# ATTron/astroz

Measured on AMD Instinct MI355X. Metric: propagations/sec, 13,478 sats x 1,440 times, at 1/2/4/8 MI355X, higher is better.
Workload: dtype f64

## Files before the change

astroz_amd/_native.py:

```python
import ctypes as C
import os

import numpy as np

_HERE = os.path.dirname(os.path.abspath(__file__))
LIB_PATH = os.environ.get("ASTROZ_AMD_LIB") or os.path.join(_HERE, "libastroz_hip.so")

WGS84, WGS72 = 0, 1
OUT_TEME, OUT_ECEF, OUT_GEODETIC, OUT_TOPOCENTRIC = 0, 1, 2, 3
SAT_MAJOR, TIME_MAJOR = 0, 1
OUTPUT_MODES = {"teme": OUT_TEME, "ecef": OUT_ECEF, "geodetic": OUT_GEODETIC, "topocentric": OUT_TOPOCENTRIC}
PASS_DTYPE = np.dtype([("t_rise_min", "<f8"), ("t_culm_min", "<f8"), ("t_set_min", "<f8"), ("max_elevation_rad", "<f8"),
                       ("rise_azimuth_rad", "<f8"), ("set_azimuth_rad", "<f8"), ("flags", "<u4"), ("grid_rise", "<u4"),
                       ("grid_culm", "<u4"), ("grid_set", "<u4")])
PASS_UP_AT_START, PASS_UP_AT_END, PASS_CUT_BY_ERROR = 1, 2, 4
ECLIPSE_DTYPE = np.dtype([("t_entry_min", "<f8"), ("t_exit_min", "<f8"), ("flags", "<u4"), ("grid_entry", "<u4"),
                          ("grid_exit", "<u4"), ("reserved", "<u4")])
ECLIPSE_IN_AT_START, ECLIPSE_IN_AT_END, ECLIPSE_CUT_BY_ERROR = 1, 2, 4
SHADOW_UMBRA, SHADOW_PENUMBRA = 0, 1
SHADOW_KINDS = {"umbra": SHADOW_UMBRA, "penumbra": SHADOW_PENUMBRA}
ACCESS_DTYPE = np.dtype([("t_start_min", "<f8"), ("t_end_min", "<f8"), ("min_range_km", "<f8"), ("flags", "<u4"),
                         ("grid_start", "<u4"), ("grid_end", "<u4"), ("grid_min_range", "<u4")])
ACCESS_OPEN_AT_START, ACCESS_OPEN_AT_END, ACCESS_CUT_BY_ERROR = 1, 2, 4
CONJUNCTION_DTYPE = np.dtype([("t_tca_min", "<f8"), ("miss_km", "<f8"), ("rel_speed_km_s", "<f8"), ("target", "<u4"),
# ... 4 lines not shown
                           ("flags", "<u4"), ("reserved", "<u4")])
COVERAGE_GAP_AT_START, COVERAGE_GAP_AT_END = 1, 2

AZ_ERR_HIP = -200
PATH_ROWS_FAST, PATH_TILES_FAST, PATH_ROWS_GENERIC, PATH_LANE_SAT, PATH_DEEP_ROWS, PATH_QUASI_UNIFORM, PATH_COLS_FAST, PATH_HOST_STEP = 1, 2, 4, 8, 16, 32, 64, 128

EXPORTS = [
    "astroz_version", "astroz_init", "astroz_deinit", "tle_parse", "tle_free",
    "tle_get_satellite_number", "tle_get_epoch", "tle_get_inclination", "tle_get_eccentricity",
    "tle_get_mean_motion", "sgp4_init", "sgp4_free", "sgp4_propagate", "sgp4_propagate_batch",
    "azh_device_count", "azh_last_error", "azh_parse_tle_lines", "azh_constellation_from_tle_text",
    "azh_constellation_from_tle_lines", "azh_constellation_from_elements", "azh_constellation_subset", "azh_constellation_free",
    "azh_num_satellites", "azh_num_sgp4", "azh_num_sdp4", "azh_get_epochs", "azh_get_status",
    "azh_get_field", "azh_propagate_host", "azh_propagate_device", "azh_propagate_device_cached", "azh_propagate_device_window",
    "azh_propagate_jd_host", "azh_synchronize", "azh_propagate_one_host", "azh_set_time_tile", "azh_set_timing", "azh_set_fast_path", "azh_set_tile_kernel", "azh_set_graphs", "azh_set_f32_arithmetic", "azh_set_f32_mode",
    "azh_last_kernel_ms", "azh_last_path", "azh_last_one_stats", "azh_last_window_tiers", "azh_last_window_ecc_tiers", "azh_set_host_copy_threads", "azh_set_host_points", "azh_get_host_points", "azh_selftest_coords", "azh_selftest_host_step", "azh_host_alloc", "azh_host_free", "azh_host_pool_stats", "azh_host_pool_trim", "azh_propagate_device_f32", "azh_propagate_device_cached_f32",
    "azh_screen_target_host", "azh_screen_target_device", "azh_coarse_screen_device", "azh_coarse_screen_host",
    "azh_screen_all_host", "azh_constellation_from_omm_json", "azh_propagate_one_device", "azh_selftest_math",
    "azh_parse_tle_text", "azh_parse_omm_json", "azh_set_parse_threads", "coords_julian_to_gmst",
    "azh_group_create_from_tle_text", "azh_group_create_from_omm_json", "azh_group_free", "azh_group_num_satellites",
    "azh_group_num_devices", "azh_group_padded_rows", "azh_group_get_epochs", "azh_group_propagate_host",
    "azh_group_propagate_allgather", "azh_group_screen_target_host", "azh_group_screen_target_device", "azh_group_shard_size",
    "azh_group_shard_rows", "azh_group_synchronize", "azh_screen_track_device", "coords_eci_to_ecef", "coords_ecef_to_geodetic",
    "orbital_hohmann", "orbital_velocity", "orbital_period", "orbital_escape_velocity",
    "azh_coords_topocentric", "azh_set_observer", "azh_find_passes_host", "azh_find_passes_device",
    "azh_find_passes_stations_host", "azh_find_passes_stations_device",
    "azh_coverage_host", "azh_coverage_device",
    "azh_sun_position_teme", "azh_selftest_sun", "azh_shadow_state", "azh_find_eclipses_host", "azh_find_eclipses_device",
    "azh_line_of_sight", "azh_find_access_host", "azh_find_access_device", "azh_find_access_track_device",
    "azh_closest_approach", "azh_find_conjunctions_host", "azh_find_conjunctions_device",
]
# ... 181 lines not shown
    L.azh_host_alloc.restype = i32
    L.azh_host_free.argtypes = [C.c_void_p]
    L.azh_host_free.restype = None
    L.azh_host_pool_stats.argtypes = [C.POINTER(C.c_size_t), C.POINTER(C.c_size_t)]
    L.azh_host_pool_stats.restype = None
    L.azh_host_pool_trim.argtypes = []
    L.azh_host_pool_trim.restype = None
    L.azh_last_path.argtypes = [vp]
    L.azh_last_path.restype = u32
    L.azh_last_one_stats.argtypes = [vp, vp, vp]
    L.azh_last_one_stats.restype = C.c_int32
    L.azh_last_window_tiers.argtypes = [vp, vp]
    L.azh_last_window_tiers.restype = C.c_int32
    L.azh_last_window_ecc_tiers.argtypes = [vp, vp]
    L.azh_last_window_ecc_tiers.restype = C.c_int32
    L.azh_propagate_device_f32.argtypes = L.azh_propagate_device.argtypes
    L.azh_propagate_device_f32.restype = i32
    L.azh_propagate_device_cached_f32.argtypes = L.azh_propagate_device_cached.argtypes
    L.azh_propagate_device_cached_f32.restype = i32
    L.azh_screen_target_host.argtypes = [vp, vp, sz, vp, sz, dbl, dbl, vp, vp]
    L.azh_screen_target_host.restype = i32
    L.azh_screen_target_device.argtypes = [vp, vp, sz, vp, sz, dbl, dbl, vp, vp, vp]
    L.azh_screen_target_device.restype = i32
    L.azh_screen_track_device.argtypes = [vp, vp, sz, vp, vp, sz, dbl, vp, vp, vp]
    L.azh_screen_track_device.restype = i32
    L.azh_coarse_screen_device.argtypes = [vp, sz, sz, i32, sz, dbl, vp, vp, vp, sz, C.POINTER(sz), vp]
    L.azh_coarse_screen_device.restype = i32
    L.azh_coarse_screen_host.argtypes = [vp, sz, sz, i32, sz, dbl, vp, vp, vp, sz, C.POINTER(sz), i32]
    L.azh_coarse_screen_host.restype = i32
    L.azh_screen_all_host.argtypes = [vp, vp, sz, vp, dbl, vp, vp, sz, C.POINTER(sz)]
# ... 422 lines not shown
        a, b = C.c_uint32(0), C.c_uint32(0)
        check(lib().azh_last_one_stats(self._h, C.byref(a), C.byref(b)), "azh_last_one_stats")
        return int(a.value), int(b.value)


    def last_window_tiers(self):
        cnt = (C.c_uint32 * 4)()
        check(lib().azh_last_window_tiers(self._h, cnt), "azh_last_window_tiers")
        return dict(zip(("general", "eps", "ecc", "rejected"), (int(x) for x in cnt)))

    def last_window_ecc_tiers(self):
        cnt = (C.c_uint32 * 3)()
        check(lib().azh_last_window_ecc_tiers(self._h, cnt), "azh_last_window_ecc_tiers")
        return dict(zip(("e1", "e2", "general"), (int(x) for x in cnt)))


class DeviceGroup:

    def __init__(self, text, devices, grav=WGS72, n_chunks=4):
        b = text.encode() if isinstance(text, str) else bytes(text)
        dv = (C.c_int32 * len(devices))(*devices)
        h = C.c_void_p()
        fn = lib().azh_group_create_from_omm_json if b.lstrip()[:1] in (b"{", b"[") else lib().azh_group_create_from_tle_text
        check(fn(b, len(b), grav, dv, len(devices), n_chunks, C.byref(h)), "azh_group_create")
        self._h = h
        self.n = lib().azh_group_num_satellites(h)
        self.n_devices = lib().azh_group_num_devices(h)
        self.padded_rows = lib().azh_group_padded_rows(h)
        self.epochs = np.empty(self.n)
        check(lib().azh_group_get_epochs(h, self.epochs.ctypes.data), "azh_group_get_epochs")
# ... 289 lines not shown
```

astroz_amd/csrc/astroz_hip.hip:

```cpp
#include "../../include/astroz_hip.h"

#include <hip/hip_runtime.h>
#include <dlfcn.h>
#include <rccl/rccl.h>

#include <algorithm>
#include <atomic>
#include <cmath>
#include <condition_variable>
#include <deque>
#include <map>
#include <cstdio>
#include <cstdlib>
#include <cstring>
#include <mutex>
#include <new>
#include <memory>
#include <string>
#include <thread>
#include <type_traits>
#include <vector>

#include "kernels.h"
#include "passes_kernel.h"
// ... 3077 lines not shown
        f.resize((size_t)pl.n_list * pl.n_seg);
    } catch (const std::bad_alloc &) {
        return AZ_ERR_HIP;
    }
    if (f.empty()) return AZ_OK;
    HIP_TRY(hipMemcpy(f.data(), pl.flag.p, f.size(), hipMemcpyDeviceToHost));
    for (unsigned char v : f) {
        if (!(v & AZ_PLAN_SET)) continue;
        if (!(v & AZ_PLAN_OK)) ++counts[AZH_WINDOW_TIER_REJECTED];
        else if (v & AZ_PLAN_ECC) ++counts[AZH_WINDOW_TIER_ECC];
        else ++counts[((v >> AZ_PLAN_TIER_SHIFT) & AZ_PLAN_TIER_MASK) ? AZH_WINDOW_TIER_EPS : AZH_WINDOW_TIER_GENERAL];
    }
    return AZ_OK;
}

int32_t azh_last_window_ecc_tiers(azh_constellation *c, uint32_t counts[AZH_WINDOW_ECC_COUNTS])
{
    if (!c || !counts) return AZ_ERR_NULL_POINTER;
    for (unsigned k = 0; k < AZH_WINDOW_ECC_COUNTS; ++k) counts[k] = 0;
    if (c->last_plan < 0 || !c->plan[c->last_plan].valid) return AZ_OK;
    const azh_constellation::FastPlan &pl = c->plan[c->last_plan];
    if (set_device(c) != AZ_OK) return AZ_ERR_HIP;
    HIP_TRY(hipDeviceSynchronize());
    std::vector<unsigned char> f;
    try {
        f.resize((size_t)pl.n_list * pl.n_seg);
    } catch (const std::bad_alloc &) {
        return AZ_ERR_HIP;
    }
    if (f.empty()) return AZ_OK;
// ... 712 lines not shown
```

astroz_amd/csrc/fast_step.h:

```cpp
#pragma once
#include <type_traits>

#include "propagate_device.h"

#define AZ_FASTK_COLD(X)                                                                                     \
    X(cc1) X(d2) X(d3) X(d4) X(nl2) X(nl3) X(nl4) X(nl5) X(eta) X(omgcof) X(xmcof) X(xd) X(bc4) X(bc5) X(ecb) X(sab)
#define AZ_FASTK_HOT(X)                                                                                      \
    X(aycof) X(xlcof) X(xnodcf) X(sinio) X(cosio) X(k_mrt) X(k_c2u) X(k_su) X(k_node) X(k_inc) X(x1mth2) X(k_rv) \
    X(sdA) X(cdA) X(sdW) X(cdW) X(tc) X(sdU) X(cdU) X(tmid) X(nodedot) X(sOc) X(cOc)
enum FastCold {
#define X(n) FC_##n,
    AZ_FASTK_COLD(X)
#undef X
    FC_NUM
};
#define AZ_FASTK_DELTA(X) X(mdot) X(argpdot) X(udot)
enum FastColdX {
    FCX_first_ = FC_NUM - 1,
#define X(n) FCX_##n,
    AZ_FASTK_DELTA(X)
#undef X
    FCX_NUM
};
#define AZ_DELTA_MAX 4.0e-6
// ... 330 lines not shown
    const double inv_pl = inv_am / (1.0 - el2);
    const double temp2 = g.half_j2 * inv_pl * inv_pl;
    ok &= temp2 <= AZ_FAST_TEMP2;
    const double a_nd = fma(fabs(k.k_node_), temp2, fma(fabs(k.nodedot_), 0.5 * fabs(t_b - t_a) + dmax, fabs(k.xnodcf_) * T * T));
    ok &= a_nd <= AZ_ROT_MED;
    if (!ok) return -1;
    if (ECC) return el <= AZ_ETIER_E1_MAX ? (int)AZ_ETIER_E1 : (el <= AZ_ETIER_E2_MAX ? (int)AZ_ETIER_E2 : (int)AZ_TIER_GENERAL);
    return eps <= AZ_TIER_EPS_MAX ? AZ_TIER_EPS : AZ_TIER_GENERAL;
}
template <bool ECC>
AZ_DEVICE bool az_fast_window_ok(const FastK &k, const AzGrav &g, double t_a, double t_b, double dmax = 0.0)
{
    return az_fast_window_tier<ECC>(k, g, t_a, t_b, dmax) >= 0;
}

#ifndef AZ_FAST_PROBE
#define AZ_FAST_PROBE(name, value)
#endif
#ifndef AZ_FAST_PROBE_KEPLER
#define AZ_FAST_PROBE_KEPLER(name, value)
#endif

template <bool VEL, bool ECC = false, int DELTA = 0, int TIER = AZ_TIER_GENERAL, class K = FastK, class RC = RotCoefLit>
AZ_DEVICE bool az_sgp4_fast_step(const K &k, const AzGrav &g, const RC &rk, double t, FastCarry &st, double r[3],
                                  double v[3], double dl = 0.0)
{
    az_pair_advance<K::SCALAR>(st.sA, st.cA, k.sdA(), k.cdA());
    az_pair_advance<K::SCALAR>(st.sW, st.cW, k.sdW(), k.cdW());
    az_pair_advance<K::SCALAR>(st.sU, st.cU, k.sdU(), k.cdU());
    double sA = st.sA, cA = st.cA, sW = st.sW, cW = st.cW;
    if constexpr ((DELTA == 1 && ECC) || DELTA == 2) {
        const double a = k.mdot() * dl, b = k.argpdot() * dl;
        if constexpr (DELTA == 2 && ECC) {
            double pa, qa;
            az_pq_16th(a, rk, pa, qa);
            az_rot_apply2(sA, cA, pa, qa);
        } else if constexpr (DELTA == 2) {
            az_rotate_tiny2(sA, cA, a, rk);
        } else {
            sA = fma(st.cA, a, st.sA); cA = fma(-st.sA, a, st.cA);
        }
        if constexpr (DELTA == 2 && ECC) az_rotate_tiny2(sW, cW, b, rk);
        else { sW = fma(st.cW, b, st.sW); cW = fma(-st.sW, b, st.cW); }
    }
    const double t2 = t * t;
    constexpr bool E1 = ECC && TIER == AZ_ETIER_E1, E2 = ECC && TIER == AZ_ETIER_E2;

    const double dm = fma(k.eta(), cA, 1.0);
    const double th = fma(k.xmcof(), dm * dm * dm, fma(k.omgcof(), t, -k.xd()));
    const double tempa = fma(-t, fma(t, fma(t, fma(t, k.d4(), k.d3()), k.d2()), k.cc1()), 1.0);
    const double dtc = t - k.tc();
    double nl = fma(k.nl2() * dtc, dtc, t2 * (t * fma(t, fma(t, k.nl5(), k.nl4()), k.nl3())));
    if constexpr (DELTA != 0) nl = fma(k.udot(), dl, nl);
    bool bad = false;
    double p, q;
    if (E1) az_fpq_small(th, rk, p, q);
    else if (ECC) az_pq_16th(th, rk, p, q);
    else az_pq_ecc_scaled(th, rk, p, q);
    const double smm = fma(cA, p, fma(sA, q, sA));
    const double sw = fma(-cW, p, fma(sW, q, sW));
    const double cw = fma(sW, p, fma(cW, q, cW));
    const double em = fma(-k.bc5(), smm, fma(-k.bc4(), t, k.ecb()));
    AZ_FAST_PROBE(th, th)
    AZ_FAST_PROBE(em, em)

    const double sqrt_am = k.sab() * fabs(tempa);
    const double am = sqrt_am * sqrt_am;
    const double omem2 = fma(-em, em, 1.0);
    const double R = az_rcp(sqrt_am * omem2);
    const double ra = R * omem2;
    const double temp = ra * R;

    const double axnl = em * cw;
    const double aynl = fma(em, sw, temp * k.aycof());
    double s = st.sU, c = st.cU;
    {
        const double eps = fma(temp * k.xlcof(), axnl, nl);
        AZ_FAST_PROBE(eps, eps)
        if constexpr (!ECC && TIER >= AZ_TIER_EPS) az_rotate_tiny2(s, c, eps, rk);
        else {
            az_pq_16th(eps, rk, p, q);
            az_rot_apply2(s, c, p, q);
        }
    }

    const double el2 = fma(axnl, axnl, aynl * aynl);
// ... 93 lines not shown

    const double est = esine * inv_1pb;
    const double sinu = inv_ome * (s - fma(axnl, est, aynl));
    const double cosu = inv_ome * (c + fma(aynl, est, -axnl));
    const double sin2u = (sinu + sinu) * cosu;
    const double cos2u = fma(-2.0 * sinu, sinu, 1.0);

    const double inv_am = ra * ra;
    const double rl = am * ome;
    const double inv_pl = inv_am * inv_omel2;
    const double temp1 = g.half_j2 * inv_pl;
    const double temp2 = temp1 * inv_pl;

    const double mrt = fma(rl, fma(k.k_mrt() * temp2, betal, 1.0), k.k_c2u() * temp1 * cos2u);
    const double t2s = temp2 * sin2u;
    const double a_nd = fma(k.k_node(), t2s, fma(k.nodedot(), t - k.tmid(), k.xnodcf() * t2));
    AZ_FAST_PROBE(a_nd, a_nd)
    double ssu = sinu, csu = cosu, sn = k.sOc(), cn = k.cOc(), si = k.sinio(), ci = k.cosio();
    az_rotate_tiny2(ssu, csu, k.k_su() * t2s, rk);
    az_pq_16th(a_nd, rk, p, q);
    az_rot_apply2(sn, cn, p, q);
    az_rotate_tiny2(si, ci, k.k_inc() * temp2 * cos2u, rk);

    const double xmx = -sn * ci, xmy = cn * ci;
    const double rs = mrt * g.radius_km;
    const double ra_s = rs * ssu, ra_c = rs * csu;
    r[0] = fma(xmx, ra_s, cn * ra_c);
    r[1] = fma(xmy, ra_s, sn * ra_c);
    r[2] = si * ra_s;
    if (VEL) {
        const double rv = ra * g.vkmpersec;
// ... 12 lines not shown
```

astroz_amd/csrc/kernels.h:

```cpp
#pragma once
#include <hip/hip_runtime.h>

#include <type_traits>

#include "init_device.h"
#include "propagate_device.h"
#include "fast_step.h"
#include "fast_step_f32.h"

#ifndef AZ_BLOCK
#define AZ_BLOCK 256
#endif
#ifndef AZ_PROP_FAST
#define AZ_PROP_FAST 1
#endif
#ifndef AZ_MIN_WAVES
#define AZ_MIN_WAVES 1
#endif
#ifndef AZ_ROWS_WAVES
#define AZ_ROWS_WAVES 3
#endif
#ifndef AZ_DEEP_WAVES
#define AZ_DEEP_WAVES 2
#endif
// ... 58 lines not shown
    const unsigned *redo_static;
    AzGrav g;
};
enum { AZ_ROW_NEAR = 0, AZ_ROW_COPY = 1, AZ_ROW_ZERO = 2 };
enum { AZ_PLAN_sOc, AZ_PLAN_cOc, AZ_PLAN_sdU, AZ_PLAN_cdU, AZ_PLAN_s1U, AZ_PLAN_c1U, AZ_PLAN_NUM };
#define AZ_PLAN_OK 1u
#define AZ_PLAN_TC 2u
#define AZ_PLAN_TIER_SHIFT 2
#define AZ_PLAN_TIER_MASK 1u
#define AZ_PLAN_ETIER_MASK 3u
#ifndef AZ_ROWS_ETIERS
#define AZ_ROWS_ETIERS 1
#endif
#define AZ_PLAN_ECC 16u
#define AZ_PLAN_SET 32u

template <class T>
__device__ __forceinline__ void az_put3(T *o, const double r[3])
{
    o[0] = (T)r[0];
    o[1] = (T)r[1];
    o[2] = (T)r[2];
}
typedef double az_d2s __attribute__((ext_vector_type(2), aligned(8)));
typedef float az_f3s __attribute__((ext_vector_type(3), aligned(4)));
#ifndef AZ_ROWS_NT
#define AZ_ROWS_NT 1
#endif
__device__ __forceinline__ void az_put3_stream(double *o, const double r[3])
{
// ... 464 lines not shown
    az_load_fast(a.el, a.n_pad, s, fl, a.inc, 0, k0);
    const double dt_mult = ecc ? 64.0 : a.dt_mult;
    if (dt_mult == 128.0) az_double_increments(k0);
    az_fast_window(a.el, a.n_pad, s, w_a, w_b, dt_mult * a.step, k0);
    az_load_fast(a.el, a.n_pad, s, fl, a.inc, 1, k1);
    az_fast_window(a.el, a.n_pad, s, w_a, w_b, a.step, k1);
    int tier = ecc ? az_fast_window_tier<true>(k0, a.g, w_a, w_b, a.delta_max) : az_fast_window_tier<false>(k0, a.g, w_a, w_b, a.delta_max);
    if (ecc && (AZ_ROWS_ETIERS == 0 || (AZ_ROWS_ETIERS == 2 && tier == AZ_ETIER_E2))) tier = min(tier, (int)AZ_TIER_GENERAL);
    bool ok = tier >= 0;
    if (!ecc && AZ_FLAG_ECLASS(fl) != 0) ok = false;
    if (!ecc && a.f32_mixed && !az_fast32p_window_ok(k0, w_a, w_b)) ok = false;
    const size_t at = (size_t)seg * a.n_list + slot;
    double *w = a.win + at * AZ_PLAN_NUM;
    w[AZ_PLAN_sOc] = k0.sOc_; w[AZ_PLAN_cOc] = k0.cOc_; w[AZ_PLAN_sdU] = k0.sdU_; w[AZ_PLAN_cdU] = k0.cdU_;
    w[AZ_PLAN_s1U] = k1.sdU_; w[AZ_PLAN_c1U] = k1.cdU_;
    a.flag[at] = (unsigned char)((ok ? AZ_PLAN_OK | ((unsigned)tier << AZ_PLAN_TIER_SHIFT) : 0u) | (k0.tc_ != 0.0 ? AZ_PLAN_TC : 0u) |
                                 (ecc ? AZ_PLAN_ECC : 0u) | AZ_PLAN_SET);
    if (!ok) {
        const unsigned k = atomicAdd(a.redo_static, 1u);
        a.redo_items[3 * (size_t)k + 0] = slot;
        a.redo_items[3 * (size_t)k + 1] = t_lo;
        a.redo_items[3 * (size_t)k + 2] = t_hi;
    }
}
__global__ void k_plan_arm(unsigned *redo_static, unsigned *c0, unsigned *c1)
{
    if (threadIdx.x == 0 && blockIdx.x == 0) *c0 = *c1 = *redo_static;
}
template <class K>
__device__ __forceinline__ bool az_plan_window(const PropArgs &p, unsigned seg, unsigned slot, double w_a, double w_b, K &k0, unsigned *tier = nullptr)
{
    const size_t at = (size_t)seg * p.plan_stride + slot;
    const double *w = p.plan_win + at * AZ_PLAN_NUM;
    const unsigned f = p.plan_flag[at];
    k0.tmid_ = 0.5 * (w_a + w_b);
    k0.tc_ = (f & AZ_PLAN_TC) ? k0.tmid_ : 0.0;
    k0.sOc_ = w[AZ_PLAN_sOc]; k0.cOc_ = w[AZ_PLAN_cOc]; k0.sdU_ = w[AZ_PLAN_sdU]; k0.cdU_ = w[AZ_PLAN_cdU];
    if (tier) *tier = (f >> AZ_PLAN_TIER_SHIFT) & ((f & AZ_PLAN_ECC) ? AZ_PLAN_ETIER_MASK : AZ_PLAN_TIER_MASK);
    return (f & AZ_PLAN_OK) != 0;
}

AZ_DEVICE double az_uniform(double x)
{
#ifdef AZ_HOST_EMUL
    return x;
#else
    return __hiloint2double(__builtin_amdgcn_readfirstlane(__double2hiint(x)),
                            __builtin_amdgcn_readfirstlane(__double2loint(x)));
#endif
}
AZ_DEVICE float az_uniform32(float x)
{
#ifdef AZ_HOST_EMUL
// ... 230 lines not shown
__global__ void __launch_bounds__(64, FRAME >= 2 ? 4 : (ECC ? AZ_ROWSF_ECC_WAVES : (FRAME == 1 || DELTA == 2 ? 5 : AZ_ROWSF_WAVES))) k_rows_fast(PropArgs p)
{
    typedef typename std::conditional<SINK == AZ_SINK_F32, float, double>::type out_t;
    const unsigned lane = threadIdx.x;
    const unsigned row = az_list_slot(p);
    [[maybe_unused]] const AzObserver obs = FRAME == 3 ? *p.obs : AzObserver{};
    if (row >= az_list_end(p)) return;
    const unsigned s = p.list[row];
    if (SINK != AZ_SINK_SCREEN && ((p.mask != nullptr && p.mask[s] == 0) || s < p.row_lo || s >= p.row_hi)) return;
    const unsigned t_lo = blockIdx.y * p.tile;
    if (t_lo >= p.n_times) return;
    const unsigned t_hi = min(t_lo + p.tile, p.n_times);
    unsigned base = t_lo;
    bool window_ok;
    unsigned tier = AZ_TIER_GENERAL;
    double best_d2 = __builtin_inf();
    unsigned best_t = 0xffffffffu;
    {
        __shared__ __attribute__((aligned(16))) double cold_lds[AZ_FAST_TABLE];
        __shared__ __attribute__((aligned(16))) out_t rows_stage[AZ_ROWS_LDS_STORE ? 2 * 64 * 3 : 4];
        const double off = az_uniform(p.offsets ? p.offsets[s] : 0.0);
        const double *__restrict__ rec = p.fast_rec + (size_t)s * FR_NUM;
        az_fill_fast_table(cold_lds, rec, lane);
        const size_t out_row = p.rows_compact ? (size_t)p.ecc_row0 + row : (size_t)s;
        out_t *prow = SINK == AZ_SINK_SCREEN ? nullptr : reinterpret_cast<out_t *>(p.pos) + out_row * p.n_times * 3;
        out_t *vrow = VEL ? reinterpret_cast<out_t *>(p.vel) + out_row * p.n_times * 3 : nullptr;
        const bool staged = AZ_ROWS_LDS_STORE && SINK != AZ_SINK_SCREEN &&
                            (((reinterpret_cast<size_t>(prow) | (VEL ? reinterpret_cast<size_t>(vrow) : 0)) & 15u) == 0);
        FastKBcast k;
        {
            const double w_a = fma((double)t_lo, p.uniform_step, p.grid_t0 + off), w_b = fma((double)(t_hi - 1), p.uniform_step, p.grid_t0 + off);
            window_ok = az_plan_window(p, blockIdx.y, row + p.redo_slot0, w_a, w_b, k, &tier);
            if (!window_ok) return;
            az_fast_rec_hot(rec, k);
            az_wave_lds_fence();
            if (DELTA && k.tc_ != 0.0 && lane == 0) cold_lds[FCX_udot] = fma(2.0 * rec[FC_nl2], k.tc_, rec[FCX_udot]);
        }
        typedef typename std::conditional<DELTA == 2, double, float>::type dl_t;
        __shared__ dl_t dl_lds[DELTA ? AZ_DELTA_SEG : 1];
        if (DELTA) {
            const dl_t *src = DELTA == 2 ? reinterpret_cast<const dl_t *>(p.delta64) : reinterpret_cast<const dl_t *>(p.delta);
#pragma unroll
            for (unsigned j = lane; j < AZ_DELTA_SEG; j += 64) dl_lds[j] = src[t_lo + j];
        }
        az_wave_lds_fence();
        const double step = p.uniform_step;
        const double t_first = p.grid_t0 + off;
        FastCarry fc;
        az_seed_fast_rec(rec, rec[FC_nl2], fma((double)(t_lo + lane) - 64.0, step, t_first), k.tc_, fc,
                         McLds{cold_lds + FCX_NUM + RC_NUM});
        __shared__ double gst_lds[FRAME ? 2 * AZ_FRAME_SEG : 2];
        if (FRAME) {
#pragma unroll
            for (unsigned j = lane; j < AZ_FRAME_SEG; j += 64) {
                const unsigned jj = min(t_lo + j, p.n_times - 1);
                gst_lds[2 * j] = p.sin_g[jj];
                gst_lds[2 * j + 1] = p.cos_g[jj];
            }
            az_wave_lds_fence();
        }
        AzRowSink sink{};
        if constexpr (SINK != AZ_SINK_SCREEN) sink = az_row_sink(prow, vrow, p.n_times);
        auto run = [&](auto tier_c, const unsigned t_end) __attribute__((always_inline)) {
        constexpr int TIER = decltype(tier_c)::value;
#pragma unroll 1
        for (; window_ok && base < t_end; base += 64) {
            const unsigned i = base + lane;
            const bool live = i < t_hi;
            double t = fma((double)i, step, t_first), dl = 0.0;
            if (DELTA) {
                dl = (double)dl_lds[i - t_lo];
                t += dl;
            }
            const double *cold_now = az_opaque_lds(cold_lds);
            k.cold = cold_now;
            const RotCoefLds rk{cold_now + FCX_NUM};
            double r[3], v[3];
#if defined(AZ_ABLATE) && AZ_ABLATE == 2
            r[0] = t; r[1] = t + 1.0; r[2] = t + 2.0; v[0] = t + 3.0; v[1] = t + 4.0; v[2] = t + 5.0;
#else
            const bool bad = az_sgp4_fast_step<VEL, ECC, DELTA, TIER>(k, p.g, rk, t, fc, r, v, dl);
            if (az_any(bad && live)) break;
#endif
            if (SINK == AZ_SINK_SCREEN) {
                const double *q = p.screen_target + (size_t)(live ? i : t_hi - 1) * 3;
                const double dx = q[0] - r[0], dy = q[1] - r[1], dz = q[2] - r[2];
                const double d2 = fma(dx, dx, fma(dy, dy, dz * dz));
                if (live && d2 < best_d2) {
                    best_d2 = d2;
                    best_t = i;
                }
                continue;
            }
            if (FRAME) {
                if (((base - t_lo) & (AZ_FRAME_SEG - 1u)) == 0u && base != t_lo) {
                    az_wave_lds_fence();
// ... 6 lines not shown
                    az_wave_lds_fence();
                }
                const unsigned jj = (i - t_lo) & (AZ_FRAME_SEG - 1u);
                const double sg = gst_lds[2 * jj], cg = gst_lds[2 * jj + 1];
                az_to_ecef(r, sg, cg);
                if (VEL) az_to_ecef(v, sg, cg);
                if (FRAME == 2) az_ecef_to_geodetic(r);
                if (FRAME == 3) az_topocentric<VEL>(r, v, obs);
            }
#if defined(AZ_ABLATE) && AZ_ABLATE == 1
            if (!(live && (r[0] + r[1] + r[2] + (VEL ? v[0] + v[1] + v[2] : 0.0)) == 1.2345e300)) continue;
#endif
            az_rows_store<VEL>(staged, base + 64 <= t_hi, live, lane, rows_stage, prow, vrow, base, r, v, sink);
        }
        };
        if constexpr (AZ_ROWS_TIERS && !ECC && FRAME == 0) run(std::integral_constant<int, AZ_TIER_EPS>(), tier == AZ_TIER_EPS ? t_hi : t_lo);
        if constexpr (AZ_ROWS_ETIERS && ECC && FRAME == 0 && DELTA != 2) {
            run(std::integral_constant<int, AZ_ETIER_E1>(), tier == AZ_ETIER_E1 ? t_hi : t_lo);
            if constexpr (AZ_ROWS_ETIERS == 1) run(std::integral_constant<int, AZ_ETIER_E2>(), tier == AZ_ETIER_E2 ? t_hi : t_lo);
        }
        run(std::integral_constant<int, AZ_TIER_GENERAL>(), t_hi);
    }
    if (SINK == AZ_SINK_SCREEN) {
        az_wave_argmin(best_d2, best_t);
        if (lane == 0) {
            p.part_d2[(size_t)blockIdx.y * p.plan_stride + row + p.redo_slot0] = best_d2;
            p.part_t[(size_t)blockIdx.y * p.plan_stride + row + p.redo_slot0] = best_t;
        }
    }
    if (ECC && base < t_hi && lane == 0) {
        const unsigned k = atomicAdd(p.redo_count, 1u);
        p.redo_items[3 * (size_t)k + 0] = row + p.redo_slot0;
        p.redo_items[3 * (size_t)k + 1] = base;
        p.redo_items[3 * (size_t)k + 2] = t_hi;
    }
}
// ... 910 lines not shown
```

bindings/zig/astroz_hip.zig:

```

pub const HipError = error{
    BadTleLength,
    BadChecksum,
    DeepSpaceNotSupported,
    InvalidEccentricity,
    SatelliteDecayed,
    ValueError,
    OutOfMemory,
    NullPointer,
    NotInitialized,
    DeviceFailure,
    Unknown,
};

pub fn check(rc: i32) HipError!void {
    return switch (rc) {
        0 => {},
        -1 => HipError.BadTleLength,
        -2 => HipError.BadChecksum,
        -10 => HipError.DeepSpaceNotSupported,
        -11 => HipError.InvalidEccentricity,
        -12 => HipError.SatelliteDecayed,
        -20 => HipError.ValueError,
        -100 => HipError.OutOfMemory,
// ... 77 lines not shown
pub extern "c" fn azh_set_f32_arithmetic(h: ?*Handle, enabled: i32) i32;
pub extern "c" fn azh_set_fast_path(h: ?*Handle, enabled: i32) i32;
pub extern "c" fn azh_set_tile_kernel(h: ?*Handle, enabled: i32) i32;
pub extern "c" fn azh_set_graphs(h: ?*Handle, enabled: i32) i32;
pub extern "c" fn azh_set_host_points(n: usize) void;
pub extern "c" fn azh_get_host_points() usize;
pub extern "c" fn azh_set_host_copy_threads(n: i32) void;
pub extern "c" fn azh_host_alloc(bytes: usize, out: *?*anyopaque) i32;
pub extern "c" fn azh_host_free(p: ?*anyopaque) void;
pub extern "c" fn azh_host_pool_stats(live_bytes: ?*usize, free_bytes: ?*usize) void;
pub extern "c" fn azh_host_pool_trim() void;
pub extern "c" fn azh_last_path(h: ?*const Handle) u32;
pub extern "c" fn azh_last_one_stats(h: ?*Handle, n_segments: ?*u32, n_handed_over: ?*u32) i32;
pub extern "c" fn azh_last_window_tiers(h: ?*Handle, counts: *[4]u32) i32;
pub extern "c" fn azh_last_window_ecc_tiers(h: ?*Handle, counts: *[3]u32) i32;
pub extern "c" fn azh_propagate_one_device(h: ?*Handle, sat_index: usize, d_tsince_min: [*]const f64, n: usize, d_pos: [*]f64,
    d_vel: ?[*]f64, d_err: ?[*]u8, stream: ?*anyopaque) i32;
pub extern "c" fn azh_selftest_math(x: [*]const f64, n: usize, out6n: [*]f64, device: i32) i32;
pub extern "c" fn azh_selftest_host_step(el: [*]const f64, n_pad: usize, sat: usize, flags: u32, grav: i32, tsince_min: [*]const f64, n: usize,
    out6n: [*]f64, err: ?[*]u8) i32;
pub extern "c" fn azh_selftest_coords(op: i32, in: *const [4]f64, out: *[5]f64) i32;

pub extern "c" fn coords_julian_to_gmst(jd: f64) f64;
pub extern "c" fn coords_eci_to_ecef(eci: *const [3]f64, gmst: f64, ecef: *[3]f64) void;
pub extern "c" fn coords_ecef_to_geodetic(ecef: *const [3]f64, lla: *[3]f64) void;
pub extern "c" fn azh_coords_topocentric(r_teme: *const [3]f64, v_teme: ?*const [3]f64, gmst: f64, observer_lla: *const [3]f64,
    aer: *[3]f64, aer_rate: ?*[3]f64) void;

pub const OUT_TOPOCENTRIC: i32 = 3;
pub const Pass = extern struct {
// ... 132 lines not shown
```

include/astroz_hip.h:

```cpp
#ifndef ASTROZ_HIP_H
#define ASTROZ_HIP_H

#include <stddef.h>
#include <stdint.h>

#ifdef __cplusplus
extern "C" {
#endif

enum {
    AZ_OK = 0,
    AZ_ERR_BAD_TLE_LENGTH = -1,
    AZ_ERR_BAD_CHECKSUM = -2,
    AZ_ERR_DEEP_SPACE_NOT_SUPPORTED = -10,
    AZ_ERR_INVALID_ECCENTRICITY = -11,
    AZ_ERR_SATELLITE_DECAYED = -12,
    AZ_ERR_VALUE = -20,
    AZ_ERR_ALLOC_FAILED = -100,
    AZ_ERR_NULL_POINTER = -101,
    AZ_ERR_NOT_INITIALIZED = -102,
    AZ_ERR_HIP = -200,
    AZ_ERR_UNKNOWN = -999
};

// ... 282 lines not shown
#define AZH_PATH_QUASI_UNIFORM 32u
#define AZH_PATH_HOST_STEP 128u
uint32_t azh_last_path(const azh_constellation *c);
int32_t azh_last_one_stats(azh_constellation *c, uint32_t *n_segments, uint32_t *n_handed_over);
#define AZH_WINDOW_TIER_GENERAL 0
#define AZH_WINDOW_TIER_EPS 1
#define AZH_WINDOW_TIER_ECC 2
#define AZH_WINDOW_TIER_REJECTED 3
#define AZH_WINDOW_TIER_COUNTS 4
int32_t azh_last_window_tiers(azh_constellation *c, uint32_t counts[AZH_WINDOW_TIER_COUNTS]);
#define AZH_WINDOW_ECC_E1 0
#define AZH_WINDOW_ECC_E2 1
#define AZH_WINDOW_ECC_GENERAL 2
#define AZH_WINDOW_ECC_COUNTS 3
int32_t azh_last_window_ecc_tiers(azh_constellation *c, uint32_t counts[AZH_WINDOW_ECC_COUNTS]);

#ifdef __cplusplus
}
#endif
#endif
```

Baseline: 97.61 billion.

## Replace per-step secular polynomials with per-64-step quadratic block expansions in LDS

For near-circular windows that pass an analytic error-bound check, the planner sets a new block flag. The rows kernel then precomputes Taylor coefficients for each 64-step block around its midpoint (am, ra, temp, nl, node, theta and eccentricity terms) and stores them in LDS. Each lane evaluates low-degree polynomials in its offset instead of the full per-time polynomials, reciprocals and divisions. This cuts per-step arithmetic, but adds an LDS table, extra template instantiations and a tolerance-bounded approximation error. A query API counts how many windows took the block path.

```diff
diff --git a/astroz_amd/_native.py b/astroz_amd/_native.py
--- a/astroz_amd/_native.py
+++ b/astroz_amd/_native.py
@@ -42,7 +42,7 @@
     "azh_num_satellites", "azh_num_sgp4", "azh_num_sdp4", "azh_get_epochs", "azh_get_status",
     "azh_get_field", "azh_propagate_host", "azh_propagate_device", "azh_propagate_device_cached", "azh_propagate_device_window",
     "azh_propagate_jd_host", "azh_synchronize", "azh_propagate_one_host", "azh_set_time_tile", "azh_set_timing", "azh_set_fast_path", "azh_set_tile_kernel", "azh_set_graphs", "azh_set_f32_arithmetic", "azh_set_f32_mode",
-    "azh_last_kernel_ms", "azh_last_path", "azh_last_one_stats", "azh_last_window_tiers", "azh_last_window_ecc_tiers", "azh_set_host_copy_threads", "azh_set_host_points", "azh_get_host_points", "azh_selftest_coords", "azh_selftest_host_step", "azh_host_alloc", "azh_host_free", "azh_host_pool_stats", "azh_host_pool_trim", "azh_propagate_device_f32", "azh_propagate_device_cached_f32",
+    "azh_last_kernel_ms", "azh_last_path", "azh_last_one_stats", "azh_last_window_tiers", "azh_last_window_ecc_tiers", "azh_last_window_blocks", "azh_set_host_copy_threads", "azh_set_host_points", "azh_get_host_points", "azh_selftest_coords", "azh_selftest_host_step", "azh_host_alloc", "azh_host_free", "azh_host_pool_stats", "azh_host_pool_trim", "azh_propagate_device_f32", "azh_propagate_device_cached_f32",
     "azh_screen_target_host", "azh_screen_target_device", "azh_coarse_screen_device", "azh_coarse_screen_host",
     "azh_screen_all_host", "azh_constellation_from_omm_json", "azh_propagate_one_device", "azh_selftest_math",
     "azh_parse_tle_text", "azh_parse_omm_json", "azh_set_parse_threads", "coords_julian_to_gmst",
@@ -254,6 +254,8 @@
     L.azh_last_window_tiers.restype = C.c_int32
     L.azh_last_window_ecc_tiers.argtypes = [vp, vp]
     L.azh_last_window_ecc_tiers.restype = C.c_int32
+    L.azh_last_window_blocks.argtypes = [vp, vp]
+    L.azh_last_window_blocks.restype = C.c_int32
     L.azh_propagate_device_f32.argtypes = L.azh_propagate_device.argtypes
     L.azh_propagate_device_f32.restype = i32
     L.azh_propagate_device_cached_f32.argtypes = L.azh_propagate_device_cached.argtypes
@@ -706,6 +708,11 @@
         check(lib().azh_last_window_ecc_tiers(self._h, cnt), "azh_last_window_ecc_tiers")
         return dict(zip(("e1", "e2", "general"), (int(x) for x in cnt)))
 
+    def last_window_blocks(self):
+        n = C.c_uint32(0)
+        check(lib().azh_last_window_blocks(self._h, C.byref(n)), "azh_last_window_blocks")
+        return int(n.value)
+
 
 class DeviceGroup:
 
diff --git a/astroz_amd/csrc/astroz_hip.hip b/astroz_amd/csrc/astroz_hip.hip
--- a/astroz_amd/csrc/astroz_hip.hip
+++ b/astroz_amd/csrc/astroz_hip.hip
@@ -3115,6 +3115,27 @@
     return AZ_OK;
 }
 
+int32_t azh_last_window_blocks(azh_constellation *c, uint32_t *n_block_windows)
+{
+    if (!c || !n_block_windows) return AZ_ERR_NULL_POINTER;
+    *n_block_windows = 0;
+    if (c->last_plan < 0 || !c->plan[c->last_plan].valid) return AZ_OK;
+    const azh_constellation::FastPlan &pl = c->plan[c->last_plan];
+    if (set_device(c) != AZ_OK) return AZ_ERR_HIP;
+    HIP_TRY(hipDeviceSynchronize());
+    std::vector<unsigned char> f;
+    try {
+        f.resize((size_t)pl.n_list * pl.n_seg);
+    } catch (const std::bad_alloc &) {
+        return AZ_ERR_HIP;
+    }
+    if (f.empty()) return AZ_OK;
+    HIP_TRY(hipMemcpy(f.data(), pl.flag.p, f.size(), hipMemcpyDeviceToHost));
+    for (unsigned char v : f)
+        if ((v & (AZ_PLAN_SET | AZ_PLAN_OK | AZ_PLAN_ECC | AZ_PLAN_BLK)) == (AZ_PLAN_SET | AZ_PLAN_OK | AZ_PLAN_BLK)) ++*n_block_windows;
+    return AZ_OK;
+}
+
 int32_t azh_last_window_ecc_tiers(azh_constellation *c, uint32_t counts[AZH_WINDOW_ECC_COUNTS])
 {
     if (!c || !counts) return AZ_ERR_NULL_POINTER;
diff --git a/astroz_amd/csrc/fast_step.h b/astroz_amd/csrc/fast_step.h
--- a/astroz_amd/csrc/fast_step.h
+++ b/astroz_amd/csrc/fast_step.h
@@ -368,17 +368,123 @@
     return az_fast_window_tier<ECC>(k, g, t_a, t_b, dmax) >= 0;
 }
 
+enum FastBlk { FB_am0, FB_am1, FB_am2, FB_ra0, FB_ra1, FB_ra2, FB_T0, FB_T1, FB_T2, FB_Tw, FB_nl0, FB_nl1, FB_nl2, FB_nl3,
+               FB_n0, FB_n1, FB_n2, FB_th0, FB_em0, FB_NUM };
+#define AZ_BLK_MAX 12
+#define AZ_BLK_TOL 2.0e-14
+struct NoBlock {
+    static constexpr bool ON = false;
+    AZ_MEMBER double x() const { return 0.0; }
+    AZ_MEMBER double operator()(int) const { return 0.0; }
+    AZ_MEMBER NoBlock after(double) const { return *this; }
+};
+struct FastBlock {
+    static constexpr bool ON = true;
+    const double *c;
+    double x_;
+    AZ_MEMBER double x() const { return x_; }
+    AZ_MEMBER double operator()(int j) const { return c[j]; }
+    AZ_MEMBER FastBlock after(double dep) const
+    {
+#ifndef AZ_HOST_EMUL
+        typedef __attribute__((address_space(3))) const double lds_cdouble;
+        lds_cdouble *q = (lds_cdouble *)c;
+        asm volatile("" : "+v"(q) : "v"(dep));
+        return FastBlock{(const double *)q, x_};
+#else
+        (void)dep;
+        return *this;
+#endif
+    }
+};
+template <class K, class W>
+AZ_DEVICE void az_fast_block_coefs(const K &k, double tb, W write)
+{
+    const double d2 = k.d2(), d3 = k.d3(), d4 = k.d4(), cc1 = k.cc1();
+    const double P = fma(-tb, fma(tb, fma(tb, fma(tb, d4, d3), d2), cc1), 1.0);
+    const double P1 = -fma(tb, fma(tb, fma(tb, 4.0 * d4, 3.0 * d3), 2.0 * d2), cc1);
+    const double P2 = -fma(tb, fma(tb, 12.0 * d4, 6.0 * d3), 2.0 * d2);
+    const double sab = k.sab(), S = sab * sab;
+    const double sq = sab * fabs(P);
+    write(FB_am0, sq * sq);
+    write(FB_am1, 2.0 * S * P * P1);
+    write(FB_am2, S * fma(P, P2, P1 * P1));
+    const double ra0 = az_rcp(sq);
+    const double iP = ra0 * sab, u = P1 * iP;
+    write(FB_ra0, ra0);
+    write(FB_ra1, -ra0 * u);
+    write(FB_ra2, ra0 * fma(u, u, -0.5 * P2 * iP));
+    const double bc4 = k.bc4();
+    const double e0 = fma(-bc4, tb, k.ecb());
+    const double gm = az_rcp(fma(-e0, e0, 1.0));
+    const double T0 = ra0 * ra0 * gm;
+    write(FB_T0, T0);
+    const double sg = bc4 * gm, es = e0 * sg;
+    write(FB_T1, -2.0 * T0 * (u + es));
+    write(FB_T2, T0 * fma(fma(3.0 * e0, e0, 1.0) * sg, sg, fma(4.0 * u, es, fma(3.0 * u, u, -P2 * iP))));
+    write(FB_Tw, -2.0 * k.bc5() * e0 * T0 * gm);
+    const double n2 = k.nl2(), n3 = k.nl3(), n4 = k.nl4(), n5 = k.nl5(), dc = tb - k.tc(), tb2 = tb * tb;
+    write(FB_nl0, fma(n2 * dc, dc, tb2 * (tb * fma(tb, fma(tb, n5, n4), n3))));
+    write(FB_nl1, fma(2.0 * n2, dc, tb2 * fma(tb, fma(tb, 5.0 * n5, 4.0 * n4), 3.0 * n3)));
+    write(FB_nl2, fma(tb, fma(tb, fma(tb, 10.0 * n5, 6.0 * n4), 3.0 * n3), n2));
+    write(FB_nl3, fma(tb, fma(tb, 10.0 * n5, 4.0 * n4), n3));
+    const double nd = k.nodedot(), xn = k.xnodcf();
+    write(FB_n0, fma(nd, tb - k.tmid(), xn * tb2));
+    write(FB_n1, fma(2.0 * xn, tb, nd));
+    write(FB_n2, xn);
+    write(FB_th0, fma(k.omgcof(), tb, -k.xd()));
+    write(FB_em0, e0);
+}
+
+enum { BQ_am, BQ_ra, BQ_T, BQ_nl, BQ_nd, BQ_NUM };
+AZ_DEVICE bool az_fast_window_blocks(const FastK &k, double t_a, double t_b, double h0, double dmax, double bnd[BQ_NUM])
+{
+    const double h = h0 + dmax;
+    const double Tb = fmax(fabs(t_a), fabs(t_b)) + h;
+    const double c1 = fabs(k.cc1_), a2 = fabs(k.d2_), a3 = fabs(k.d3_), a4 = fabs(k.d4_);
+    const double da = Tb * fma(Tb, fma(Tb, fma(Tb, a4, a3), a2), c1);
+    const double D1 = fma(Tb, fma(Tb, fma(Tb, 4.0 * a4, 3.0 * a3), 2.0 * a2), c1);
+    const double D2 = fma(Tb, fma(Tb, 12.0 * a4, 6.0 * a3), 2.0 * a2);
+    const double D3 = fma(Tb, 24.0 * a4, 6.0 * a3);
+    const double Pmax = 1.0 + da, iP = 1.0 / (1.0 - da), iP2 = iP * iP, iP3 = iP2 * iP;
+    const double b4 = fabs(k.bc4_), b5 = fabs(k.bc5_);
+    const double emx = fabs(k.ecb_) + fma(b4, Tb, b5);
+    bool ok = (da <= 0.5) & (emx <= 0.9);
+    const double h3 = h * h * h * (1.0 / 6.0);
+    bnd[BQ_am] = fma(fma(6.0 * D1, D2, 2.0 * Pmax * D3) * iP2, h3, 2.0e-15);
+    bnd[BQ_ra] = fma(fma(6.0 * D1 * D1 * D1, iP2 * iP2, fma(6.0 * D1 * D2, iP3, D3 * iP2)) * Pmax, h3, 2.0e-15);
+    const double iS = 1.0 / (k.sab_ * k.sab_);
+    const double A0 = iP2 * iS, A1 = 2.0 * D1 * iP3 * iS, A2 = fma(6.0 * D1 * D1, iP2 * iP2, 2.0 * D2 * iP3) * iS;
+    const double F0 = 1.0 / fma(-emx, emx, 1.0), F1 = 2.0 * emx * F0 * F0, F2 = fma(6.0 * emx, emx, 2.0) * F0 * F0 * F0;
+    const double A3 = fma(24.0 * D1 * D1 * D1, iP2 * iP3, fma(18.0 * D1 * D2, iP2 * iP2, 2.0 * D3 * iP3)) * iS;
+    const double F3 = 24.0 * emx * fma(emx, emx, 1.0) * F0 * F0 * F0 * F0;
+    const double T3 = fma(A3, F0, b4 * fma(3.0 * A2, F1, b4 * fma(3.0 * A1, F2, A0 * F3 * b4)));
+    const double dTw = b5 * fma(A1, F1, A0 * F2 * b4);
+    const double errT = fma(T3, h3, fma(dTw, h, 0.5 * A0 * F2 * b5 * b5)) + 3.0e-15 * A0 * F0;
+    bnd[BQ_T] = errT * fmax(fabs(k.aycof_), fabs(k.xlcof_) * emx);
+    const double n4 = fabs(k.nl4_), n5 = fabs(k.nl5_), h2 = h * h;
+    bnd[BQ_nl] = fma(h2 * h2, fma(5.0 * n5, Tb, n4) + n5 * h, 2.0e-16);
+    bnd[BQ_nd] = 2.0e-16;
+#pragma unroll
+    for (int q = 0; q < BQ_NUM; ++q) ok &= bnd[q] <= AZ_BLK_TOL;
+    return ok;
+}
+
 #ifndef AZ_FAST_PROBE
 #define AZ_FAST_PROBE(name, value)
 #endif
 #ifndef AZ_FAST_PROBE_KEPLER
 #define AZ_FAST_PROBE_KEPLER(name, value)
 #endif
-
-template <bool VEL, bool ECC = false, int DELTA = 0, int TIER = AZ_TIER_GENERAL, class K = FastK, class RC = RotCoefLit>
+#ifndef AZ_FAST_PROBE_BLOCK
+#define AZ_FAST_PROBE_BLOCK(name, value)
+#endif
+
+template <bool VEL, bool ECC = false, int DELTA = 0, int TIER = AZ_TIER_GENERAL, class K = FastK, class RC = RotCoefLit, class B = NoBlock>
 AZ_DEVICE bool az_sgp4_fast_step(const K &k, const AzGrav &g, const RC &rk, double t, FastCarry &st, double r[3],
-                                  double v[3], double dl = 0.0)
-{
+                                  double v[3], double dl = 0.0, const B &b = B())
+{
+    static_assert(!B::ON || (!ECC && DELTA <= 1), "the block form: near-circular bodies, exact and tight grids");
     az_pair_advance<K::SCALAR>(st.sA, st.cA, k.sdA(), k.cdA());
     az_pair_advance<K::SCALAR>(st.sW, st.cW, k.sdW(), k.cdW());
     az_pair_advance<K::SCALAR>(st.sU, st.cU, k.sdU(), k.cdU());
@@ -401,11 +507,16 @@
     constexpr bool E1 = ECC && TIER == AZ_ETIER_E1, E2 = ECC && TIER == AZ_ETIER_E2;
 
     const double dm = fma(k.eta(), cA, 1.0);
-    const double th = fma(k.xmcof(), dm * dm * dm, fma(k.omgcof(), t, -k.xd()));
-    const double tempa = fma(-t, fma(t, fma(t, fma(t, k.d4(), k.d3()), k.d2()), k.cc1()), 1.0);
+    double th, tempa = 1.0, nl = 0.0;
+    if constexpr (B::ON) {
+        th = fma(k.xmcof(), dm * dm * dm, fma(k.omgcof(), b.x(), b(FB_th0)));
+    } else {
+    th = fma(k.xmcof(), dm * dm * dm, fma(k.omgcof(), t, -k.xd()));
+    tempa = fma(-t, fma(t, fma(t, fma(t, k.d4(), k.d3()), k.d2()), k.cc1()), 1.0);
     const double dtc = t - k.tc();
-    double nl = fma(k.nl2() * dtc, dtc, t2 * (t * fma(t, fma(t, k.nl5(), k.nl4()), k.nl3())));
-    if constexpr (DELTA != 0) nl = fma(k.udot(), dl, nl);
+    nl = fma(k.nl2() * dtc, dtc, t2 * (t * fma(t, fma(t, k.nl5(), k.nl4()), k.nl3())));
+    }
+    if constexpr (DELTA != 0 && !B::ON) nl = fma(k.udot(), dl, nl);
     bool bad = false;
     double p, q;
     if (E1) az_fpq_small(th, rk, p, q);
@@ -414,16 +525,29 @@
     const double smm = fma(cA, p, fma(sA, q, sA));
     const double sw = fma(-cW, p, fma(sW, q, sW));
     const double cw = fma(sW, p, fma(cW, q, cW));
-    const double em = fma(-k.bc5(), smm, fma(-k.bc4(), t, k.ecb()));
+    const double em = fma(-k.bc5(), smm, B::ON ? fma(-k.bc4(), b.x(), b(FB_em0)) : fma(-k.bc4(), t, k.ecb()));
     AZ_FAST_PROBE(th, th)
     AZ_FAST_PROBE(em, em)
 
+    double am = 0.0, ra = 0.0, temp;
+    if constexpr (B::ON) {
+        temp = fma(b(FB_Tw), smm, fma(b.x(), fma(b.x(), b(FB_T2), b(FB_T1)), b(FB_T0)));
+        nl = fma(b.x(), fma(b.x(), fma(b.x(), b(FB_nl3), b(FB_nl2)), b(FB_nl1)), b(FB_nl0));
+        if constexpr (DELTA != 0) nl = fma(k.udot(), dl, nl);
+        am = fma(b.x(), fma(b.x(), b(FB_am2), b(FB_am1)), b(FB_am0));
+        ra = fma(b.x(), fma(b.x(), b(FB_ra2), b(FB_ra1)), b(FB_ra0));
+    } else {
     const double sqrt_am = k.sab() * fabs(tempa);
-    const double am = sqrt_am * sqrt_am;
+    am = sqrt_am * sqrt_am;
     const double omem2 = fma(-em, em, 1.0);
     const double R = az_rcp(sqrt_am * omem2);
-    const double ra = R * omem2;
-    const double temp = ra * R;
+    ra = R * omem2;
+    temp = ra * R;
+    }
+    AZ_FAST_PROBE_BLOCK(temp, temp)
+    AZ_FAST_PROBE_BLOCK(nl, nl)
+    AZ_FAST_PROBE_BLOCK(am, am)
+    AZ_FAST_PROBE_BLOCK(ra, ra)
 
     const double axnl = em * cw;
     const double aynl = fma(em, sw, temp * k.aycof());
@@ -547,7 +671,15 @@
 
     const double mrt = fma(rl, fma(k.k_mrt() * temp2, betal, 1.0), k.k_c2u() * temp1 * cos2u);
     const double t2s = temp2 * sin2u;
-    const double a_nd = fma(k.k_node(), t2s, fma(k.nodedot(), t - k.tmid(), k.xnodcf() * t2));
+    double nd;
+    if constexpr (B::ON) {
+        const B b3 = b.after(ome);
+        nd = fma(b.x(), fma(b3(FB_n2), b.x(), b3(FB_n1)), b3(FB_n0));
+    } else {
+        nd = fma(k.nodedot(), t - k.tmid(), k.xnodcf() * t2);
+    }
+    AZ_FAST_PROBE_BLOCK(nd, nd)
+    const double a_nd = fma(k.k_node(), t2s, nd);
     AZ_FAST_PROBE(a_nd, a_nd)
     double ssu = sinu, csu = cosu, sn = k.sOc(), cn = k.cOc(), si = k.sinio(), ci = k.cosio();
     az_rotate_tiny2(ssu, csu, k.k_su() * t2s, rk);
diff --git a/astroz_amd/csrc/kernels.h b/astroz_amd/csrc/kernels.h
--- a/astroz_amd/csrc/kernels.h
+++ b/astroz_amd/csrc/kernels.h
@@ -96,6 +96,10 @@
 #endif
 #define AZ_PLAN_ECC 16u
 #define AZ_PLAN_SET 32u
+#define AZ_PLAN_BLK 64u
+#ifndef AZ_ROWS_BLOCKS
+#define AZ_ROWS_BLOCKS 1
+#endif
 
 template <class T>
 __device__ __forceinline__ void az_put3(T *o, const double r[3])
@@ -590,8 +594,13 @@
     double *w = a.win + at * AZ_PLAN_NUM;
     w[AZ_PLAN_sOc] = k0.sOc_; w[AZ_PLAN_cOc] = k0.cOc_; w[AZ_PLAN_sdU] = k0.sdU_; w[AZ_PLAN_cdU] = k0.cdU_;
     w[AZ_PLAN_s1U] = k1.sdU_; w[AZ_PLAN_c1U] = k1.cdU_;
+    bool blk = false;
+    if (AZ_ROWS_BLOCKS && ok && !ecc && tile <= 64u * AZ_BLK_MAX && a.delta_max <= AZ_DELTA_MAX) {
+        double bnd[BQ_NUM];
+        blk = az_fast_window_blocks(k0, w_a, w_b, 31.5 * fabs(a.step), a.delta_max, bnd);
+    }
     a.flag[at] = (unsigned char)((ok ? AZ_PLAN_OK | ((unsigned)tier << AZ_PLAN_TIER_SHIFT) : 0u) | (k0.tc_ != 0.0 ? AZ_PLAN_TC : 0u) |
-                                 (ecc ? AZ_PLAN_ECC : 0u) | AZ_PLAN_SET);
+                                 (ecc ? AZ_PLAN_ECC : 0u) | (blk ? AZ_PLAN_BLK : 0u) | AZ_PLAN_SET);
     if (!ok) {
         const unsigned k = atomicAdd(a.redo_static, 1u);
         a.redo_items[3 * (size_t)k + 0] = slot;
@@ -604,7 +613,8 @@
     if (threadIdx.x == 0 && blockIdx.x == 0) *c0 = *c1 = *redo_static;
 }
 template <class K>
-__device__ __forceinline__ bool az_plan_window(const PropArgs &p, unsigned seg, unsigned slot, double w_a, double w_b, K &k0, unsigned *tier = nullptr)
+__device__ __forceinline__ bool az_plan_window(const PropArgs &p, unsigned seg, unsigned slot, double w_a, double w_b, K &k0, unsigned *tier = nullptr,
+                                               bool *blk = nullptr)
 {
     const size_t at = (size_t)seg * p.plan_stride + slot;
     const double *w = p.plan_win + at * AZ_PLAN_NUM;
@@ -613,6 +623,7 @@
     k0.tc_ = (f & AZ_PLAN_TC) ? k0.tmid_ : 0.0;
     k0.sOc_ = w[AZ_PLAN_sOc]; k0.cOc_ = w[AZ_PLAN_cOc]; k0.sdU_ = w[AZ_PLAN_sdU]; k0.cdU_ = w[AZ_PLAN_cdU];
     if (tier) *tier = (f >> AZ_PLAN_TIER_SHIFT) & ((f & AZ_PLAN_ECC) ? AZ_PLAN_ETIER_MASK : AZ_PLAN_TIER_MASK);
+    if (blk) *blk = (f & AZ_PLAN_BLK) != 0;
     return (f & AZ_PLAN_OK) != 0;
 }
 
@@ -873,6 +884,8 @@
     unsigned base = t_lo;
     bool window_ok;
     unsigned tier = AZ_TIER_GENERAL;
+    constexpr bool BLK = AZ_ROWS_BLOCKS && AZ_ROWS_TIERS && !ECC && FRAME == 0 && DELTA <= 1 && SINK != AZ_SINK_SCREEN;
+    bool blk = false;
     double best_d2 = __builtin_inf();
     unsigned best_t = 0xffffffffu;
     {
@@ -889,8 +902,9 @@
         FastKBcast k;
         {
             const double w_a = fma((double)t_lo, p.uniform_step, p.grid_t0 + off), w_b = fma((double)(t_hi - 1), p.uniform_step, p.grid_t0 + off);
-            window_ok = az_plan_window(p, blockIdx.y, row + p.redo_slot0, w_a, w_b, k, &tier);
+            window_ok = az_plan_window(p, blockIdx.y, row + p.redo_slot0, w_a, w_b, k, &tier, BLK ? &blk : nullptr);
             if (!window_ok) return;
+            blk = blk && t_hi - t_lo <= 64u * AZ_BLK_MAX;
             az_fast_rec_hot(rec, k);
             az_wave_lds_fence();
             if (DELTA && k.tc_ != 0.0 && lane == 0) cold_lds[FCX_udot] = fma(2.0 * rec[FC_nl2], k.tc_, rec[FCX_udot]);
@@ -905,6 +919,18 @@
         az_wave_lds_fence();
         const double step = p.uniform_step;
         const double t_first = p.grid_t0 + off;
+        __shared__ __attribute__((aligned(16))) double blk_lds[BLK ? AZ_BLK_MAX * FB_NUM : 2];
+        [[maybe_unused]] const double blk_x = ((double)lane - 31.5) * step;
+        if constexpr (BLK) {
+            if (blk) {
+                k.cold = cold_lds;
+                double *dst = blk_lds + (lane < (unsigned)AZ_BLK_MAX ? lane : 0u) * FB_NUM;
+                az_fast_block_coefs(k, fma((double)(t_lo + 64u * lane) + 31.5, step, t_first), [&](int j, double v) {
+                    if (lane < (unsigned)AZ_BLK_MAX) dst[j] = v;
+                });
+                az_wave_lds_fence();
+            }
+        }
         FastCarry fc;
         az_seed_fast_rec(rec, rec[FC_nl2], fma((double)(t_lo + lane) - 64.0, step, t_first), k.tc_, fc,
                          McLds{cold_lds + FCX_NUM + RC_NUM});
@@ -920,8 +946,9 @@
         }
         AzRowSink sink{};
         if constexpr (SINK != AZ_SINK_SCREEN) sink = az_row_sink(prow, vrow, p.n_times);
-        auto run = [&](auto tier_c, const unsigned t_end) __attribute__((always_inline)) {
+        auto run = [&](auto tier_c, auto blk_c, const unsigned t_end) __attribute__((always_inline)) {
         constexpr int TIER = decltype(tier_c)::value;
+        constexpr bool BLKF = decltype(blk_c)::value;
 #pragma unroll 1
         for (; window_ok && base < t_end; base += 64) {
             const unsigned i = base + lane;
@@ -938,7 +965,19 @@
 #if defined(AZ_ABLATE) && AZ_ABLATE == 2
             r[0] = t; r[1] = t + 1.0; r[2] = t + 2.0; v[0] = t + 3.0; v[1] = t + 4.0; v[2] = t + 5.0;
 #else
-            const bool bad = az_sgp4_fast_step<VEL, ECC, DELTA, TIER>(k, p.g, rk, t, fc, r, v, dl);
+            bool bad;
+            if constexpr (BLKF) {
+                double x = blk_x;
+                if constexpr (DELTA != 0) {
+                    unsigned ln = lane;
+                    asm volatile("" : "+v"(ln));
+                    x = fma((double)ln - 31.5, step, dl);
+                }
+                const FastBlock fb{az_opaque_lds(blk_lds + ((base - t_lo) >> 6) * FB_NUM), x};
+                bad = az_sgp4_fast_step<VEL, ECC, DELTA, TIER>(k, p.g, rk, t, fc, r, v, dl, fb);
+            } else {
+                bad = az_sgp4_fast_step<VEL, ECC, DELTA, TIER>(k, p.g, rk, t, fc, r, v, dl);
+            }
             if (az_any(bad && live)) break;
 #endif
             if (SINK == AZ_SINK_SCREEN) {
@@ -975,12 +1014,16 @@
             az_rows_store<VEL>(staged, base + 64 <= t_hi, live, lane, rows_stage, prow, vrow, base, r, v, sink);
         }
         };
-        if constexpr (AZ_ROWS_TIERS && !ECC && FRAME == 0) run(std::integral_constant<int, AZ_TIER_EPS>(), tier == AZ_TIER_EPS ? t_hi : t_lo);
+        typedef std::false_type exact_c;
+        if constexpr (BLK) {
+            run(std::integral_constant<int, AZ_TIER_EPS>(), std::true_type(), blk && tier == AZ_TIER_EPS ? t_hi : t_lo);
+            run(std::integral_constant<int, AZ_TIER_GENERAL>(), std::true_type(), blk ? t_hi : t_lo);
+        } else if constexpr (AZ_ROWS_TIERS && !ECC && FRAME == 0) run(std::integral_constant<int, AZ_TIER_EPS>(), exact_c(), tier == AZ_TIER_EPS ? t_hi : t_lo);
         if constexpr (AZ_ROWS_ETIERS && ECC && FRAME == 0 && DELTA != 2) {
-            run(std::integral_constant<int, AZ_ETIER_E1>(), tier == AZ_ETIER_E1 ? t_hi : t_lo);
-            if constexpr (AZ_ROWS_ETIERS == 1) run(std::integral_constant<int, AZ_ETIER_E2>(), tier == AZ_ETIER_E2 ? t_hi : t_lo);
-        }
-        run(std::integral_constant<int, AZ_TIER_GENERAL>(), t_hi);
+            run(std::integral_constant<int, AZ_ETIER_E1>(), exact_c(), tier == AZ_ETIER_E1 ? t_hi : t_lo);
+            if constexpr (AZ_ROWS_ETIERS == 1) run(std::integral_constant<int, AZ_ETIER_E2>(), exact_c(), tier == AZ_ETIER_E2 ? t_hi : t_lo);
+        }
+        run(std::integral_constant<int, AZ_TIER_GENERAL>(), exact_c(), t_hi);
     }
     if (SINK == AZ_SINK_SCREEN) {
         az_wave_argmin(best_d2, best_t);
diff --git a/bindings/zig/astroz_hip.zig b/bindings/zig/astroz_hip.zig
--- a/bindings/zig/astroz_hip.zig
+++ b/bindings/zig/astroz_hip.zig
@@ -115,6 +115,7 @@
 pub extern "c" fn azh_last_one_stats(h: ?*Handle, n_segments: ?*u32, n_handed_over: ?*u32) i32;
 pub extern "c" fn azh_last_window_tiers(h: ?*Handle, counts: *[4]u32) i32;
 pub extern "c" fn azh_last_window_ecc_tiers(h: ?*Handle, counts: *[3]u32) i32;
+pub extern "c" fn azh_last_window_blocks(h: ?*Handle, n_block_windows: *u32) i32;
 pub extern "c" fn azh_propagate_one_device(h: ?*Handle, sat_index: usize, d_tsince_min: [*]const f64, n: usize, d_pos: [*]f64,
     d_vel: ?[*]f64, d_err: ?[*]u8, stream: ?*anyopaque) i32;
 pub extern "c" fn azh_selftest_math(x: [*]const f64, n: usize, out6n: [*]f64, device: i32) i32;
diff --git a/include/astroz_hip.h b/include/astroz_hip.h
--- a/include/astroz_hip.h
+++ b/include/astroz_hip.h
@@ -320,6 +320,7 @@
 #define AZH_WINDOW_ECC_GENERAL 2
 #define AZH_WINDOW_ECC_COUNTS 3
 int32_t azh_last_window_ecc_tiers(azh_constellation *c, uint32_t counts[AZH_WINDOW_ECC_COUNTS]);
+int32_t azh_last_window_blocks(azh_constellation *c, uint32_t *n_block_windows);
 
 #ifdef __cplusplus
 }
```

Result: no change. 96.91 billion (median of 2 runs) (-0.7%).
